# torognes/vsearch

Hardware: AMD Instinct MI355X
Metric: GCUPS (useful DP cells/s of the search16 global-alignment path: DP + traceback + CIGAR) (higher is better)
Workload: dtype int16

## Files before the change

### vsearch_amd/csrc/vsx_device.hip

```cpp
#include <hip/hip_runtime.h>
#include <type_traits>
#include <cstdlib>
#include <atomic>
#include "vsx_internal.h"

typedef unsigned int u32;
typedef unsigned int u32x4 __attribute__((ext_vector_type(4)));
typedef unsigned int u32x3 __attribute__((ext_vector_type(3)));
typedef short s2 __attribute__((ext_vector_type(2)));
typedef unsigned short us2 __attribute__((ext_vector_type(2)));

#define DEV __device__ __forceinline__
struct __attribute__((aligned(4))) Pair2 { unsigned int x, y; };

#define SIGN2 0x80008000u

DEV s2 S2(u32 x) { return __builtin_bit_cast(s2, x); }
DEV us2 U2(u32 x) { return __builtin_bit_cast(us2, x); }
DEV u32 UI(s2 x) { return __builtin_bit_cast(u32, x); }
DEV u32 UI(us2 x) { return __builtin_bit_cast(u32, x); }

DEV u32 sadd(u32 a, u32 b) { return UI(__builtin_elementwise_add_sat(S2(a), S2(b))); }
DEV u32 ssub(u32 a, u32 b) { return UI(__builtin_elementwise_sub_sat(S2(a), S2(b))); }
DEV u32 pmax(u32 a, u32 b) { return UI(__builtin_elementwise_max(S2(a), S2(b))); }
DEV u32 pmin(u32 a, u32 b) { return UI(__builtin_elementwise_min(S2(a), S2(b))); }
DEV u32 pminu(u32 a, u32 b) { return UI(__builtin_elementwise_min(U2(a), U2(b))); }
DEV u32 pmaxu(u32 a, u32 b) { return UI(__builtin_elementwise_max(U2(a), U2(b))); }
DEV u32 psubw(u32 a, u32 b) { return UI((us2) (U2(a) - U2(b))); }
DEV u32 pmad(u32 a, u32 b, u32 c) { return UI((us2) (U2(a) * U2(b) + U2(c))); }
DEV u32 pashr15(u32 a) { return UI((s2) (S2(a) >> (s2){15, 15})); }
DEV u32 bfi(u32 mask, u32 a, u32 b) { return (a & mask) | (b & ~mask); }
DEV u32 a_pk_minu(u32 a, u32 b) { u32 r; asm("v_pk_min_u16 %0, %1, %2" : "=v"(r) : "v"(a), "s"(b)); return r; }
DEV u32 a_pk_mad(u32 a, u32 b, u32 c) { u32 r; asm("v_pk_mad_u16 %0, %1, %2, %3" : "=v"(r) : "v"(a), "v"(b), "s"(c)); return r; }
DEV u32 a_bfi(u32 mask, u32 a, u32 b) { u32 r; asm("v_bfi_b32 %0, %1, %2, %3" : "=v"(r) : "s"(mask), "v"(a), "v"(b)); return r; }
DEV u32 a_bfi_v(u32 mask, u32 a, u32 b) { u32 r; asm("v_bfi_b32 %0, %1, %2, %3" : "=v"(r) : "v"(mask), "v"(a), "v"(b)); return r; }
DEV u32 a_lshr1(u32 a) { u32 r; asm("v_lshrrev_b32 %0, 1, %1" : "=v"(r) : "v"(a)); return r; }
DEV u32 a_pk_ashr15(u32 a) { u32 r; asm("v_pk_ashrrev_i16 %0, 15, %1 op_sel_hi:[0,1]" : "=v"(r) : "v"(a)); return r; }
DEV u32 funnel(u32 acc, u32 d) { return a_bfi(SIGN2, d, a_lshr1(acc)); }
DEV u32 pack16(int v) { const u32 x = (u32) v & 0xffffu; return x | (x << 16); }

DEV u32 dpp_shr1(u32 feed, u32 src) { return (u32) __builtin_amdgcn_update_dpp((int) feed, (int) src, 0x111, 0xF, 0xF, false); }
DEV u32 dpp_rol1(u32 src) { return (u32) __builtin_amdgcn_update_dpp((int) src, (int) src, 0x12F, 0xF, 0xF, false); }


#define VSX_COLCK_G 64
#define VSX_COLCK_DW(R_, lane_, block_) ((((size_t) ((lane_) / VSX_COLCK_G) * (size_t) ((2 * (R_)) / 4) + (size_t) (block_)) * VSX_COLCK_G + (size_t) ((lane_) % VSX_COLCK_G)) * 4)
#define VSX_RB 1
#define VSX_ROWCK_PAIR_DW(TILT_) ((TILT_) ? 192 : 256)
#define VSX_COLCK_NBH(RT_) (((RT_) + ((RT_) + 1) / 2 + 3) / 4)
#define VSX_COLCK_NB(R_, TILT_) ((TILT_) ? (VSX_MID(R_, true) ? 2 * VSX_COLCK_NBH((R_) / 2) : ((R_) + ((R_) + 1) / 2 + 3) / 4) : (2 * (R_)) / 4)
#ifndef VSX_CK_TASKMAJOR
#define VSX_CK_TASKMAJOR 1
#endif
#define VSX_CK_SLOT(TILT_, g_, l_) (((TILT_) && VSX_CK_TASKMAJOR) ? ((l_) * 4 + (g_)) : ((g_) * 16 + (l_)))
#ifndef VSX_COLCK_CG
#define VSX_COLCK_CG 64
#endif
#define VSX_CKT_BLOCK_DW 768
#define VSX_COLCK_NCHUNK(R_) ((VSX_COLCK_NB(R_, true) + 2) / 3)
#define VSX_COLCK_CDW(NB_, lane_, block_) ((((size_t) ((lane_) / VSX_COLCK_CG) * (size_t) (NB_) + (size_t) (block_)) * VSX_COLCK_CG + (size_t) ((lane_) % VSX_COLCK_CG)) * 4)
#ifndef VSX_FWD_WAVES
#define VSX_FWD_WAVES(R_, TILT_) ((R_) <= 16 ? 4 : ((R_) <= 24 ? 3 : 2))
#endif
#ifndef VSX_FWD_WAVES_ONE
#define VSX_FWD_WAVES_ONE(R_, TILT_) ((R_) == 26 ? 3 : VSX_FWD_WAVES(R_, TILT_))
#endif
typedef _Float16 f16x2 __attribute__((ext_vector_type(2)));
DEV u32 pk_max3_bits(u32 a, u32 b, u32 c)
{
  const f16x2 x = __builtin_bit_cast(f16x2, a), y = __builtin_bit_cast(f16x2, b), z = __builtin_bit_cast(f16x2, c);
  return __builtin_bit_cast(u32, __builtin_elementwise_maximum(__builtin_elementwise_maximum(x, y), z));
}
#ifndef VSX_FWD_WAVES_NQ
#define VSX_FWD_WAVES_NQ(R_, NQ_) ((NQ_) == 4 ? 2 : ((R_) <= 24 ? 3 : 2))
#endif
template <int R, bool GENERIC, bool TRACK, bool CKPT, bool TILT = false, bool MAX3 = false, int NQ = 1, bool PAIR = false, bool ONE = false>
__global__ void __launch_bounds__(PAIR ? 256 : 64) __attribute__((amdgpu_waves_per_eu(NQ == 1 ? (ONE ? VSX_FWD_WAVES_ONE(R, TILT) : VSX_FWD_WAVES(R, TILT)) : VSX_FWD_WAVES_NQ(R, NQ), 8)))
vsx_forward_kernel(const VsxDevParams P, const VsxTask * __restrict__ tasks,
                   const uint8_t * __restrict__ qc, const uint8_t * __restrict__ tc,
                   u32 * __restrict__ dir, uint2 * strip, VsxSlotOut * __restrict__ slot_out, const u32 ntasks)
{
  constexpr int ND = (R + 3) / 4;
  constexpr bool TOPPAD = CKPT && GENERIC && !TRACK;
  static_assert(!TILT || TOPPAD, "tilted coordinates exist for the TOPPAD class only");
  const int tl = TILT ? P.tilt : 0;
  static_assert(!MAX3 || TILT, "the MAX3 arithmetic is a sub-class of TILT");
  constexpr u32 BIAS16 = MAX3 ? 0x3E00u : (TILT ? 0x8000u : 0u);
  constexpr u32 BIAS = BIAS16 * 0x10001u;
  constexpr u32 CK_REBIAS = 0u;
  auto bpack = [](int v) -> u32 { return pack16(v + (int) BIAS16); };
  auto vadd = [](u32 a, u32 b) -> u32 { return TILT ? a + b : sadd(a, b); };
  auto vsubk = [](u32 a, u32 b) -> u32 { return TILT ? a - b : ssub(a, b); };
  auto vsub = [](u32 a, u32 b) -> u32 { return TILT ? psubw(a, b) : ssub(a, b); };
  auto vmax = [](u32 a, u32 b) -> u32 { return TILT ? pmaxu(a, b) : pmax(a, b); };
  constexpr bool MIDCK = VSX_MID(R, TILT);
  constexpr int RT = MIDCK ? R / 2 : R;
  constexpr bool CKST = TILT && (VSX_CKT != 0);
  static_assert(!(MAX3 && CKST), "the transposed A/B layout predates the MAX3 class");
  constexpr bool QPL = TILT && (VSX_QPL != 0);
  constexpr bool QP8 = CKST || QPL;
  constexpr int RP = (R + 3) & ~3;
  static_assert(NQ == 1 || NQ == 2 || NQ == 4, "tasks per wave");
  static_assert(NQ == 1 || (TILT && VSX_QPL != 0 && !VSX_CKT), "the sparse-task classes exist for the look-ahead TILT kernels only");
  static_assert(!PAIR || (NQ == 1 && TILT && VSX_QPL != 0 && VSX_FEED2 != 0 && !VSX_CKT && GENERIC), "the pair-profile classes extend the FEED2 look-ahead kernels");
  constexpr int WPB = PAIR ? 4 : 1;
  constexpr int QPBYTES = 16 * 16 * RP;
  constexpr int RPP = ((RP / 4) & 1) ? RP : RP + 4;
  __shared__ __attribute__((aligned(16))) u32 PPf[PAIR ? 16 * 16 * RPP : 4];
  __shared__ __attribute__((aligned(16))) int16_t QP[(GENERIC && !PAIR) ? (QP8 ? (NQ * QPBYTES) / 2 : 16 * 16 * R) : 8];
  uint8_t * const QPb = reinterpret_cast<uint8_t *>(QP);
  __shared__ __attribute__((aligned(16))) u32 RS[CKST ? 64 * 12 : 4];
  constexpr int FSZ = (TILT && VSX_QPL ? 2 : 1) * 4 * 16;
  __shared__ uint4 FEED4a[FSZ * WPB];
  __shared__ u32 FEEDFa[FSZ * WPB], FEEDN[GENERIC ? 1 : 4 * 16];
  constexpr bool FEED2 = (VSX_FEED2 != 0) && TOPPAD && (TILT && (VSX_QPL != 0));
  __shared__ uint2 FEEDBa[FEED2 ? 2 * 4 * 16 * WPB : 1];

  const int wv = PAIR ? __builtin_amdgcn_readfirstlane((int) (threadIdx.x >> 6)) : 0;
  uint4 * const FEED4 = FEED4a + wv * FSZ;
  u32 * const FEEDF = FEEDFa + wv * FSZ;
  uint2 * const FEEDB = FEEDBa + (FEED2 ? wv * FSZ : 0);
  const int lane = PAIR ? (int) (threadIdx.x & 63) : (int) threadIdx.x;
  const int gw = lane >> 4;
  constexpr int GPT = 4 / NQ;
  const int sq = (NQ == 1) ? 0 : gw / GPT;
  const int g = (NQ == 1) ? gw : gw % GPT;
  const int l = lane & 15;
  const u32 tix = PAIR ? blockIdx.x * 4u + (u32) wv : ((NQ == 1) ? blockIdx.x : blockIdx.x * (u32) NQ + (u32) sq);
  const bool sub_on = (NQ == 1 && !PAIR) ? true : (tix < ntasks);
  const VsxTask & T = tasks[sub_on ? tix : ntasks - 1];
  uint8_t * const QPl = reinterpret_cast<uint8_t *>(QP) + ((NQ == 1) ? 0 : sq * QPBYTES);

  const int Q = (int) T.qlen;
  const int total_lanes = (Q + R - 1) / R;
  const int rcnt0 = Q - (total_lanes - 1) * R;
  const int rc0 = __builtin_amdgcn_readfirstlane(rcnt0);
  static_assert(!PAIR || ONE, "the pair-profile classes are planned for single-strip queries only");
  const int nstrips = (NQ == 1 && !ONE) ? (total_lanes + 15) >> 4 : 1;
  const int steps = (NQ == 1) ? (int) T.steps : __builtin_amdgcn_readfirstlane((int) T.steps);

  const int DA = sub_on ? (int) T.tlen[2 * g] : 0;
  const int DB = sub_on ? (int) T.tlen[2 * g + 1] : 0;
  const int DpA = (DA + 3) & ~3;
  const int DpB = (DB + 3) & ~3;
  const int Dpg = DpA > DpB ? DpA : DpB;
  const uint8_t * __restrict__ tA = tc + T.toff[2 * g];
  const uint8_t * __restrict__ tB = tc + T.toff[2 * g + 1];
  const uint8_t * __restrict__ qq = qc + T.qoff;

  const u32 qrt_i_pk = pack16(P.qrt_i);
  u32 hmin = 0, hmax = 0;
  u32 score = 0;
  u32 lv1 = 0xFFFFFFFFu, leave = 0;

  for (int s = 0; s < nstrips; ++s)
    {
      const int L = 16 * s + l;
      const bool lane_on = (L < total_lanes) && (Dpg > 0);
      const bool first = (L == 0);
      const int pad = TOPPAD ? R - rcnt0 : 0;
      const int i0 = first ? -pad : rcnt0 + (L - 1) * R;

      if (GENERIC)
        {
          __syncthreads();
          if (PAIR)
            {
              for (int idx = (int) threadIdx.x; idx < 16 * 16 * RP; idx += 256)
                {
                  const int pr = idx / (16 * RP), row = idx % (16 * RP);
                  const int Lr = 16 * s + row / RP, rr = row % RP;
                  int va = 0, vb = 0;
                  if (rr < R)
                    {
                      if (Lr == 0 && rr < pad) va = vb = -P.top_step + 2 * tl;
                      else if (Lr < total_lanes)
                        {
                          const int gi = (Lr == 0) ? rr - pad : rcnt0 + (Lr - 1) * R + rr;
                          const int qs = (int) qq[gi];
                          va = P.matrix[(1 << (pr >> 2)) * 16 + qs];
                          vb = P.matrix[(1 << (pr & 3)) * 16 + qs];
                        }
                    }
                  PPf[(pr * 16 + row / RP) * RPP + rr] = ((u32) va & 0xffu) | (((u32) vb & 0xffu) << 16);
                }
            }
          else if (QP8)
            {
              constexpr int LPT = 64 / NQ;
              for (int idx = (NQ == 1) ? lane : lane % LPT; idx < 16 * 16 * RP; idx += LPT)
                {
                  const int code = idx / (16 * RP), row = idx % (16 * RP);
                  const int Lr = 16 * s + row / RP, rr = row % RP;
                  int v = 0;
                  if (rr < R)
                    {
                      if (Lr == 0 && rr < pad) v = -P.top_step + 2 * tl;
                      else if (Lr < total_lanes)
                        {
                          const int gi = (Lr == 0) ? rr - pad : rcnt0 + (Lr - 1) * R + rr;
                          v = P.matrix[code * 16 + (int) qq[gi]];
                        }
                    }
                  QPl[idx] = (uint8_t) v;
                }
            }
          else
          for (int idx = lane; idx < 16 * 16 * R; idx += 64)
            {
              const int code = idx / (16 * R), row = idx % (16 * R);
              const int Lr = 16 * s + row / R, rr = row % R;
              int v = 0;
              if (TOPPAD && Lr == 0 && rr < pad) v = -P.top_step + 2 * tl;
              else if (Lr < total_lanes && (TOPPAD || !(Lr == 0 && rr >= rcnt0)))
                {
                  const int gi = (Lr == 0) ? rr - pad : rcnt0 + (Lr - 1) * R + rr;
                  v = P.matrix[code * 16 + (int) qq[gi]];
                }
              QP[idx] = (int16_t) v;
            }
          __syncthreads();
        }

      u32 hprev[R];
      u32 hnext[R];
      u32 E[R];
      u32 ac[R];
#pragma unroll
      for (int r = 0; r < R; ++r)
        {
          int i = i0 + r;
          const bool dummy = TOPPAD && first && r < pad;
          if (i > Q - 1) i = Q - 1;
          if (i < 0) i = 0;
          const u32 a = qq[i];
          ac[r] = a | (a << 16);
          u32 hl = bpack(P.hleft[i]);
          u32 e0 = vsub(hl, (i < Q - 1) ? P.qrq_i_pk : P.qrq_r_pk);
          if (dummy)
            {
              const int sh = (r - pad - 1) * tl;
              hl = bpack(((r == pad - 1) ? 0 : -P.top_open) + sh);
              e0 = vsub(bpack(-P.top_open - P.top_step + sh), P.qrq_i_pk);
            }
          hprev[r] = hl;
          hnext[r] = hl;
          E[r] = e0;
        }
      u32 diag = first ? bpack(((TOPPAD && pad > 0) ? -P.top_open : 0) - (pad + 2) * tl) : bpack(P.hleft[i0 - 1]);
      const bool lastpos = (L == total_lanes - 1);
      const u32 qrq_last = lastpos ? P.qrq_r_pk : P.qrq_i_pk;
      const u32 rq_last = lastpos ? P.rq_r_pk : P.rq_i_pk;

      u32 sym = 0, nd = 0, qrt = 0, rt = 0;
      u32 symf = 0;
      u32 outH = 0, outF = 0;
      u32 f_sym = 0, f_nd = 0, f_qrt = 0, f_rt = 0, f_H = 0, f_F = 0;
      u32 rawA = 0, rawB = 0;
      int rawH = 0;
      uint2 rawS = make_uint2(0, 0);
      const uint2 * strip_in = strip + T.strip_off + (size_t) (((s + 1) & 1) * 4 + g) * (size_t) steps;
      uint2 * strip_outp = strip + T.strip_off + (size_t) ((s & 1) * 4 + g) * (size_t) steps;

      auto prefetch = [&](int blk) {
        const int c = 16 * blk + l;
        rawA = (c < DA) ? (u32) tA[c] : 0u;
        rawB = (c < DB) ? (u32) tB[c] : 0u;
        if (s == 0) rawH = P.htop[c];
        else if (c < Dpg) rawS = strip_in[c];
      };
      prefetch(0);

      auto build_feed = [&](int blk) __attribute__((always_inline)) {
              const int c = 16 * blk + l;
              auto mne = [&](u32 code) -> int {
                const bool unamb = (code != 0) && ((code & (code - 1)) == 0);
                return unamb ? P.mismatch : ((P.n_mismatch && code == 15) ? P.mismatch : 0);
              };
              const u32 ndA = (u32) (mne(rawA) - P.match) & 0xffffu;
              const u32 ndB = (u32) (mne(rawB) - P.match) & 0xffffu;
              const u32 qA = (u32) ((c < DA - 1) ? P.qrt_i : P.qrt_r) & 0xffffu;
              const u32 qB = (u32) ((c < DB - 1) ? P.qrt_i : P.qrt_r) & 0xffffu;
              const u32 rA = (u32) ((c < DA - 1) ? P.rt_i : P.rt_r) & 0xffffu;
              const u32 rB = (u32) ((c < DB - 1) ? P.rt_i : P.rt_r) & 0xffffu;
              const u32 sA = rawA | ((c == DA - 1) ? 0x100u : 0u) | ((c < DpA) ? 0x200u : 0u);
              const u32 sB = rawB | ((c == DB - 1) ? 0x100u : 0u) | ((c < DpB) ? 0x200u : 0u);
              f_sym = sA | (sB << 16);
              f_nd = ndA | (ndB << 16);
              f_qrt = qA | (qB << 16);
              f_rt = rA | (rB << 16);
              if (s == 0)
                {
                  f_H = bpack(rawH - pad * tl);
                  f_F = vsub(f_H, f_qrt);
                }
              else
                {
                  f_H = rawS.x;
                  f_F = rawS.y;
                }
              const int fo = QPL ? (blk & 1) * 64 : 0;
              if (FEED2)
                {
                  const u32 f_off = PAIR ? (((rawA >> 1) - (rawA >> 3)) * 4u + ((rawB >> 1) - (rawB >> 3))) * (u32) (16 * RPP * 4)
                                         : (rawA * (u32) (16 * RP) | ((rawB * (u32) (16 * RP)) << 16));
                  FEED4[fo + gw * 16 + l] = make_uint4(f_off, f_sym, f_H, f_F);
                  FEEDB[fo + gw * 16 + l] = make_uint2(f_qrt, f_rt);
                }
              else
                {
                  FEED4[fo + gw * 16 + l] = make_uint4(f_sym, f_qrt, f_rt, f_H);
                  FEEDF[fo + gw * 16 + l] = f_F;
                }
              if (!GENERIC) FEEDN[gw * 16 + l] = f_nd;
              prefetch(blk + 1);
      };
      constexpr int PD = RP / 4;
      u32 profA[2][(QPL && !PAIR) ? PD : 1], profB[2][(QPL && !PAIR) ? PD : 1];
      auto load_profile = [&](u32 (&buf)[2][(QPL && !PAIR) ? PD : 1], u32 sy) __attribute__((always_inline)) {
        if (PAIR) return;
        const u32 cd = sy & 0x000F000Fu;
        constexpr int QPA = (RP % 16 == 0) ? 16 : ((RP % 8 == 0) ? 8 : 4);
        if (FEED2)
          {
            const uint8_t * pa = QPl + l * RP + (sy & 0xFFFFu);
            const uint8_t * pb = QPl + l * RP + (sy >> 16);
            constexpr int PDN = (QPL && !PAIR) ? PD : 1;
            if constexpr (PAIR) { }
            else if constexpr (QPA == 16)
              {
#pragma unroll
                for (int k = 0; k < PDN; k += 4)
                  {
                    const uint4 va = *reinterpret_cast<const uint4 *>(pa + 4 * k), vb = *reinterpret_cast<const uint4 *>(pb + 4 * k);
                    buf[0][k] = va.x; buf[0][k + 1] = va.y; buf[0][k + 2] = va.z; buf[0][k + 3] = va.w;
                    buf[1][k] = vb.x; buf[1][k + 1] = vb.y; buf[1][k + 2] = vb.z; buf[1][k + 3] = vb.w;
                  }
              }
            else if constexpr (QPA == 8)
              {
#pragma unroll
                for (int k = 0; k < PDN; k += 2)
                  {
                    const uint2 va = *reinterpret_cast<const uint2 *>(pa + 4 * k), vb = *reinterpret_cast<const uint2 *>(pb + 4 * k);
                    buf[0][k] = va.x; buf[0][k + 1] = va.y;
                    buf[1][k] = vb.x; buf[1][k + 1] = vb.y;
                  }
              }
            else
              {
#pragma unroll
                for (int k = 0; k < PDN; ++k)
                  { buf[0][k] = reinterpret_cast<const u32 *>(pa)[k]; buf[1][k] = reinterpret_cast<const u32 *>(pb)[k]; }
              }
            return;
          }
        const u32 * a = reinterpret_cast<const u32 *>(QPl + (cd & 0xFu) * (16 * RP) + l * RP);
        const u32 * b = reinterpret_cast<const u32 *>(QPl + (cd >> 16) * (16 * RP) + l * RP);
#pragma unroll
        for (int k = 0; k < ((QPL && !PAIR) ? PD : 1); ++k) { buf[0][k] = a[k]; buf[1][k] = b[k]; }
      };
      if (QPL)
        {
          build_feed(0);
          sym = dpp_shr1(FEED4[gw * 16].x, 0u);
          load_profile(profA, sym);
        }

      const uint4 * const feed4_g = FEED4 + gw * 16;
      const u32 * const feedf_g = FEEDF + gw * 16;
      u32 pendH = 0, pendF = 0;
      u32 jpk_run = 0;
      u32 pendMH = 0, pendMF = 0, curMH = 0, curMF = 0;
      bool pend_on = false;
      const size_t ck_rowdw = ((((size_t) nstrips * steps + 1) & ~(size_t) 1) >> 1) * VSX_ROWCK_PAIR_DW(TILT);
      const size_t ck_nblk = ((size_t) steps + 15) >> 4;
      constexpr int CK_LANE_DW = TILT ? 3 : 4;
      constexpr size_t CK_COL_DW = TILT ? (size_t) 64 * 4 * VSX_COLCK_NB(R, true) : (size_t) 64 * (2 * R);
      const int ck_slot = VSX_CK_SLOT(TILT, gw, l);
      u32 * const rck_base = dir + T.dir_off + ((((size_t) s * steps) >> 1) * 64 + ck_slot) * CK_LANE_DW;
      u32 * const cck_base = dir + T.dir_off + ck_rowdw + (size_t) s * ck_nblk * CK_COL_DW;
      u32 * const mck_base = dir + T.dir_off + ck_rowdw + (size_t) nstrips * ck_nblk * CK_COL_DW
                             + ((((size_t) s * steps) >> 1) * 64 + ck_slot) * CK_LANE_DW;
      u32 * const rck_blk = dir + T.dir_off + (((size_t) s * steps) >> 3) * VSX_CKT_BLOCK_DW;
      u32 * const cck_blk = dir + T.dir_off + (((size_t) nstrips * steps) >> 3) * VSX_CKT_BLOCK_DW
                            + (size_t) s * ck_nblk * VSX_COLCK_NCHUNK(R) * VSX_CKT_BLOCK_DW;
      auto flush_block = [&](u32 * gdst) __attribute__((always_inline)) {
        __syncthreads();
#pragma unroll
        for (int k = 0; k < 3; ++k)
          {
            const u32x4 v = *reinterpret_cast<const u32x4 *>(RS + (k * 64 + lane) * 4);
            __builtin_nontemporal_store(v, reinterpret_cast<u32x4 *>(gdst + (k * 64 + lane) * 4));
          }
        __syncthreads();
      };

      auto step = [&](const int t, u32 (&hin)[R], u32 (&hout)[R], u32 (&pc)[2][(QPL && !PAIR) ? PD : 1], u32 (&pn)[2][(QPL && !PAIR) ? PD : 1],
                      auto interior_tag, auto odd_tag, auto steady_tag) __attribute__((always_inline)) {
          constexpr bool INTERIOR = decltype(interior_tag)::value;
          constexpr bool ODD = decltype(odd_tag)::value;
          constexpr bool STEADY = decltype(steady_tag)::value;
          u32 symn = 0;
          u32 pp[PAIR ? RP : 1];
          if (PAIR)
            {
              const u32 * ppa = PPf + (sym >> 2) + l * RPP;
#pragma unroll
              for (int k = 0; k < (PAIR ? RP : 0); k += 4)
                {
                  const uint4 v = *reinterpret_cast<const uint4 *>(ppa + k);
                  pp[k] = v.x; pp[k + 1] = v.y; pp[k + 2] = v.z; pp[k + 3] = v.w;
                }
            }
          if (QPL) { if ((t & 15) == 15) build_feed((t >> 4) + 1); }
          else if ((t & 15) == 0) build_feed(t >> 4);

          const int fo = QPL ? ((t >> 4) & 1) * 64 : 0;
          const u32 fslot = (u32) (fo + (t & 15));
          const uint4 fv = feed4_g[fslot];
          const u32 fF = FEED2 ? fv.w : feedf_g[fslot];
          if (QPL)
            {
              const int t1 = t + 1;
              symn = dpp_shr1(feed4_g[(u32) (((t1 >> 4) & 1) * 64 + (t1 & 15))].x, sym);
              load_profile(pn, symn);
            }
          else sym = dpp_shr1(fv.x, sym);
          if (!GENERIC) nd = dpp_shr1(FEEDN[gw * 16 + (t & 15)], nd);
          if (!INTERIOR)
            {
              if (FEED2)
                {
                  const uint2 fb = FEEDB[fo + gw * 16 + (t & 15)];
                  qrt = dpp_shr1(fb.x, qrt); rt = dpp_shr1(fb.y, rt);
                  symf = dpp_shr1(fv.y, symf);
                }
              else { qrt = dpp_shr1(fv.y, qrt); rt = dpp_shr1(fv.z, rt); }
            }
          const u32 inH = dpp_shr1(FEED2 ? fv.z : fv.w, outH);
          const u32 inF = dpp_shr1(fF, outF);

          const int j = t - l;
          const bool active = STEADY ? true : (lane_on && j >= 0 && j < Dpg);
          if (active)
            {
              const u32 code = sym & 0x000F000Fu;
              const int16_t * qpA = QP + (code & 0xFu) * (16 * R) + l * R;
              const int16_t * qpB = QP + (code >> 16) * (16 * R) + l * R;
              u32 pa = 0, pb = 0;
              u32 Hd = diag;
              u32 F = inF;
              u32 smn = 0x7FFF7FFFu, smx = 0x80008000u;
              u32 acc = 0, h2 = 0;
              u32 capH = 0, capF = 0, capmn = 0, capmx = 0;
              u32 dw[ND];
              u32 lastL = 0, lastEL = 0;
              u32 midH = 0, midF = 0;
              auto rows = [&](auto shared_tag) __attribute__((always_inline)) {
              constexpr bool SHARED = decltype(shared_tag)::value;
              constexpr bool LASTFAST = MAX3 && SHARED && CKPT;
#pragma unroll
              for (int r = 0; r < R; ++r)
                {
                  u32 V;
                  if (PAIR) V = pp[r];
                  else if (GENERIC && QP8)
                    {
                      if ((r & 3) == 0)
                        {
                          if (QPL) { pa = pc[0][r >> 2]; pb = pc[1][r >> 2]; }
                          else
                            {
                              pa = *reinterpret_cast<const u32 *>(QPb + (code & 0xFu) * (16 * RP) + l * RP + r);
                              pb = *reinterpret_cast<const u32 *>(QPb + (code >> 16) * (16 * RP) + l * RP + r);
                            }
                        }
                      V = __builtin_amdgcn_perm(pb, pa, 0x0C040C00u + 0x00010001u * (u32) (r & 3));
                    }
                  else if (GENERIC)
                    {
                      if (R % 2 == 0)
                        {
                          if ((r & 3) == 0 && r + 3 < R)
                            {
                              typedef typename std::conditional<R % 4 == 0, uint2, Pair2>::type Rows4;
                              const Rows4 va = *reinterpret_cast<const Rows4 *>(qpA + r);
                              const Rows4 vb = *reinterpret_cast<const Rows4 *>(qpB + r);
                              pa = va.x; pb = vb.x;
                              ac[r + 1] = va.y; ac[r + 2] = vb.y;
                            }
                          else if ((r & 3) == 0)
                            {
                              pa = *reinterpret_cast<const u32 *>(qpA + r);
                              pb = *reinterpret_cast<const u32 *>(qpB + r);
                            }
                          else if ((r & 3) == 2) { pa = ac[r - 1]; pb = ac[r]; }
                          V = (r & 1) ? __builtin_amdgcn_perm(pb, pa, 0x07060302u) : __builtin_amdgcn_perm(pb, pa, 0x05040100u);
                        }
                      else V = (u32) (uint16_t) qpA[r] | ((u32) (uint16_t) qpB[r] << 16);
                    }
                  else V = a_pk_mad(a_pk_minu(ac[r] ^ code, 0x00010001u), nd, P.match_pk);
                  const u32 h0 = vadd(Hd, V);
                  const bool ONE_MAX = MAX3 && (r < R - 1 || LASTFAST);
                  const u32 h1 = ONE_MAX ? 0u : vmax(h0, F);
                  h2 = ONE_MAX ? pk_max3_bits(h0, F, E[r]) : vmax(h1, E[r]);
                  if (TRACK) { smn = pmin(smn, h2); smx = pmax(smx, h2); }
                  Hd = hin[r];
                  hout[r] = h2;
                  const u32 qrq = (r == R - 1) ? qrq_last : P.qrq_i_pk;
                  const u32 rq = (r == R - 1) ? rq_last : P.rq_i_pk;
                  const u32 he = (r < R - 1) ? vsubk(h2, qrq) : vsub(h2, qrq);
                  const u32 hf = (SHARED && r < R - 1) ? he : vsub(h2, qrt);
                  const u32 f = (TILT && INTERIOR) ? F : vsub(F, rt);
                  const u32 e = (TILT && INTERIOR && r < R - 1) ? E[r] : vsub(E[r], rq);
                  if (CKPT && r == R - 1) { lastL = LASTFAST ? 0u : vsub(h1, E[r]); lastEL = vsub(he, e); }
                  if (!CKPT)
                    {
                      const u32 dU = ssub(h0, F);
                      const u32 dL = ssub(h1, E[r]);
                      const u32 dEU = ssub(hf, f);
                      const u32 dEL = ssub(he, e);
                      acc = funnel(funnel(funnel(funnel(acc, dU), dL), dEU), dEL);
                      if ((r & 3) == 3 || r == R - 1) dw[r >> 2] = acc;
                    }
                  F = vmax(f, hf);
                  E[r] = vmax(e, he);
                  if (MIDCK && r == RT - 1) { midH = h2; midF = F; }
                  if (!TOPPAD && __builtin_expect(rc0 == r + 1, 0)) { capH = h2; capF = F; capmn = smn; capmx = smx; }
                }
              };
              if (INTERIOR) rows(std::true_type {});
              else rows(std::false_type {});
              const u32 hl = (!TOPPAD && first) ? capH : h2;
              F = (!TOPPAD && first) ? capF : F;
              smn = (!TOPPAD && first) ? capmn : smn;
              smx = (!TOPPAD && first) ? capmx : smx;
              outH = hl;
              outF = F;
              diag = inH;
              if (CKPT)
                {
                  const u32 jpk = STEADY ? jpk_run : ((u32) j | ((u32) j << 16));
                  if (STEADY) jpk_run += 0x00010001u;
                  if (!INTERIOR)
                    {
                      const u32 atlast = a_pk_ashr15((FEED2 ? symf : sym) << 7);
                      leave = a_bfi_v(atlast, a_bfi_v(a_pk_ashr15(lastL), lv1, jpk), leave);
                    }
                  lv1 = a_bfi_v(a_pk_ashr15((MAX3 && INTERIOR) ? lastEL : (lastL | lastEL)), lv1, jpk);
                }

              if (TRACK)
                {
                  const u32 vm = a_pk_ashr15(sym << 6);
                  hmin = pmin(hmin, a_bfi_v(vm, smn, 0x7FFF7FFFu));
                  hmax = pmax(hmax, a_bfi_v(vm, smx, 0x80008000u));
                }
              if (!INTERIOR)
                {
                  const u32 lm = a_pk_ashr15((FEED2 ? symf : sym) << 7);
                  score = a_bfi_v(lm, hl, score);
                }

              const size_t gt = (size_t) s * steps + t;
              if (CKPT)
                {
                  if (!ODD) { pendH = outH; pendF = outF; }
                  if (MIDCK) { if (!ODD) { pendMH = midH; pendMF = midF; } else { curMH = midH; curMF = midF; } }
                }
              else
                {
                  u32 * dp = dir + T.dir_off + (((gt >> 2) * 64 + lane) * 4 + (gt & 3)) * ND;
                  if (ND == 4) *reinterpret_cast<uint4 *>(dp) = make_uint4(dw[0], dw[1], dw[2], dw[3]);
                  else if (ND == 2) *reinterpret_cast<uint2 *>(dp) = make_uint2(dw[0], dw[1]);
                  else
                    {
#pragma unroll
                      for (int w = 0; w < ND; ++w) dp[w] = dw[w];
                    }
                }
              if (l == 15 && s + 1 < nstrips) strip_outp[j] = make_uint2(outH, outF);
            }
          if (CKPT && CKST)
            {
              if (!ODD) pend_on = active;
              else
                {
                  const u32 dpk = __builtin_amdgcn_perm(psubw(outH, outF), psubw(pendH, pendF), 0x06040200u);
                  u32 * rs = RS + ck_slot * 12;
                  const int i = t & 7;
                  *reinterpret_cast<uint2 *>(rs + (i - 1)) = make_uint2(pendH, outH);
                  rs[8 + (i >> 1)] = dpk;
                  if (i == 7) flush_block(rck_blk + (size_t) (t >> 3) * VSX_CKT_BLOCK_DW);
                }
            }
          else if (CKPT)
            {
              if (!ODD) pend_on = active;
              else if (pend_on || active)
                {
                  if (TILT && !CKST)
                    {
                      const u32 dpk = __builtin_amdgcn_perm(psubw(outH, outF), psubw(pendH, pendF), 0x06040200u);
                      __builtin_nontemporal_store((u32x3) {pendH + CK_REBIAS, outH + CK_REBIAS, dpk}, reinterpret_cast<u32x3 *>(rck_base + (size_t) (t >> 1) * 192));
                      if (MIDCK)
                        {
                          const u32 dpm = __builtin_amdgcn_perm(psubw(curMH, curMF), psubw(pendMH, pendMF), 0x06040200u);
                          __builtin_nontemporal_store((u32x3) {pendMH + CK_REBIAS, curMH + CK_REBIAS, dpm}, reinterpret_cast<u32x3 *>(mck_base + (size_t) (t >> 1) * 192));
                        }
                    }
                  else
                    __builtin_nontemporal_store((u32x4) {pendH, pendF, outH, outF}, reinterpret_cast<u32x4 *>(rck_base + (size_t) (t >> 1) * 256));
                }
            }
          if (CKPT && (t & 15) == 15)
            {
              u32 * cb = cck_base + (size_t) (t >> 4) * CK_COL_DW;
              if (TILT)
                {
                  constexpr int NF = R + (R + 1) / 2;
                  constexpr int NFH = RT + (RT + 1) / 2, ZH = 4 * VSX_COLCK_NBH(RT);
                  auto flatc = [&](int z) -> u32 {
                    if (MIDCK)
                      {
                        const int hh = z / ZH, zz = z % ZH, r00 = hh * RT;
                        if (zz < RT) return hout[r00 + zz] + CK_REBIAS;
                        if (zz < NFH)
                          {
                            const int r0 = r00 + 2 * (zz - RT), r1 = (r0 + 1 < r00 + RT) ? r0 + 1 : r0;
                            return __builtin_amdgcn_perm(psubw(hout[r1], E[r1]), psubw(hout[r0], E[r0]), 0x06040200u);
                          }
                        return 0u;
                      }
                    if (z < R) return hout[z] + CK_REBIAS;
                    if (z < NF)
                      {
                        const int r0 = 2 * (z - R), r1 = r0 + 1 < R ? r0 + 1 : r0;
                        return __builtin_amdgcn_perm(psubw(hout[r1], E[r1]), psubw(hout[r0], E[r0]), 0x06040200u);
                      }
                    return 0u;
                  };
                  if (CKST)
                    {
                      constexpr int NBC = VSX_COLCK_NB(R, true);
#pragma unroll
                      for (int c = 0; c < VSX_COLCK_NCHUNK(R); ++c)
                        {
#pragma unroll
                          for (int pc = 0; pc < 3; ++pc)
                            {
                              const int z = 4 * (3 * c + pc);
                              if (3 * c + pc < NBC)
                                *reinterpret_cast<u32x4 *>(RS + ck_slot * 12 + pc * 4) = (u32x4) {flatc(z), flatc(z + 1), flatc(z + 2), flatc(z + 3)};
                            }
                          flush_block(cck_blk + ((size_t) (t >> 4) * VSX_COLCK_NCHUNK(R) + c) * VSX_CKT_BLOCK_DW);
                        }
                    }
                  else
                    {
#pragma unroll
                  for (int z = 0; z < 4 * VSX_COLCK_NB(R, true); z += 4)
                    __builtin_nontemporal_store((u32x4) {flatc(z), flatc(z + 1), flatc(z + 2), flatc(z + 3)}, reinterpret_cast<u32x4 *>(cb + VSX_COLCK_CDW(VSX_COLCK_NB(R, true), ck_slot, z >> 2)));
                    }
                }
              else if (R % 2 == 0)
                {
                  auto flat = [&](int z) -> u32 { return z < R ? hout[z] : E[z - R]; };
#pragma unroll
                  for (int z = 0; z < 2 * R; z += 4)
                    __builtin_nontemporal_store((u32x4) {flat(z), flat(z + 1), flat(z + 2), flat(z + 3)}, reinterpret_cast<u32x4 *>(cb + VSX_COLCK_DW(R, lane, z >> 2)));
                }
              else
                {
                  u32 * cp = cb + lane * (2 * R);
#pragma unroll
                  for (int x = 0; x < R; ++x) { cp[x] = hout[x]; cp[R + x] = E[x]; }
                }
            }
          if (QPL) sym = symn;
      };
      int t_switch = 0;
      if (CKPT && P.share_sub)
        {
          int dmin = 0x7fffffff;
          if (DA > 0 && DA < dmin) dmin = DA;
          if (DB > 0 && DB < dmin) dmin = DB;
#pragma unroll
          for (int m = 32; m >= 1; m >>= 1) { const int o = __shfl_xor(dmin, m, 64); dmin = o < dmin ? o : dmin; }
          t_switch = __builtin_amdgcn_readfirstlane(dmin == 0x7fffffff ? 0 : dmin - 1) & ~1;
          if (t_switch > steps) t_switch = steps & ~1;
        }
      int t = 0;
      qrt = qrt_i_pk; rt = pack16(P.rt_i);
      for (; t < t_switch && (TRACK || t < 16); t += 2)
        {
          step(t, hprev, hnext, profA, profB, std::true_type {}, std::false_type {}, std::false_type {});
          step(t + 1, hnext, hprev, profB, profA, std::true_type {}, std::true_type {}, std::false_type {});
        }
      if (!TRACK)
        for (jpk_run = (u32) (t - l) * 0x00010001u; t < t_switch; t += 2)
          {
            step(t, hprev, hnext, profA, profB, std::true_type {}, std::false_type {}, std::true_type {});
            step(t + 1, hnext, hprev, profB, profA, std::true_type {}, std::true_type {}, std::true_type {});
          }
      for (; t < steps; t += 2)
        {
          step(t, hprev, hnext, profA, profB, std::false_type {}, std::false_type {}, std::false_type {});
          step(t + 1, hnext, hprev, profB, profA, std::false_type {}, std::true_type {}, std::false_type {});
        }

      if (s + 1 < nstrips)
        {
          __builtin_amdgcn_fence(__ATOMIC_RELEASE, "agent");
          __builtin_amdgcn_fence(__ATOMIC_ACQUIRE, "agent");
        }
    }

#pragma unroll
  for (int m = 8; m >= 1; m >>= 1)
    {
      hmin = pmin(hmin, (u32) __shfl_xor((int) hmin, m, 16));
      hmax = pmax(hmax, (u32) __shfl_xor((int) hmax, m, 16));
    }
  const int l_last = (total_lanes - 1) & 15;
  score = (u32) __shfl((int) score, l_last, 16);
  leave = (u32) __shfl((int) leave, l_last, 16);
  if (l == 0)
    {
      const int mnA = (int16_t) (hmin & 0xffff), mnB = (int16_t) (hmin >> 16);
      const int mxA = (int16_t) (hmax & 0xffff), mxB = (int16_t) (hmax >> 16);
      VsxSlotOut oA, oB;
      score = psubw(score, BIAS);
      oA.score = (int16_t) ((int) (int16_t) (score & 0xffff) - (DA > 0 ? (Q + DA - 2) * tl : 0));
      oB.score = (int16_t) ((int) (int16_t) (score >> 16) - (DB > 0 ? (Q + DB - 2) * tl : 0));
      oA.leave = (uint16_t) (leave & 0xffff); oB.leave = (uint16_t) (leave >> 16); oA.pad = 0; oB.pad = 0;
      oA.overflow = (mnA <= P.smin || mxA >= 32767) ? 1 : 0;
      oB.overflow = (mnB <= P.smin || mxB >= 32767) ? 1 : 0;
      if (sub_on)
        {
          slot_out[(size_t) tix * VSX_TASK_SLOTS + 2 * g] = oA;
          slot_out[(size_t) tix * VSX_TASK_SLOTS + 2 * g + 1] = oB;
        }
    }
}

__global__ void __launch_bounds__(256)
vsx_traceback_kernel(const VsxDevParams P, const VsxTask * __restrict__ tasks,
                     const u32 * __restrict__ pair_slot, const u32 * __restrict__ pair_ids, u32 npairs,
                     const uint8_t * __restrict__ qc, const uint8_t * __restrict__ tc,
                     const u32 * __restrict__ dir, const VsxSlotOut * __restrict__ slot,
                     u32 * __restrict__ slab, const uint64_t * __restrict__ slab_off,
                     u32 * __restrict__ runs, uint64_t runs_capacity, unsigned long long * cursor,
                     VsxPairOut * __restrict__ out)
{
  const u32 k = blockIdx.x * blockDim.x + threadIdx.x;
  if (k >= npairs) return;
  const u32 ts = pair_slot[k];
  const u32 task = ts >> 3, sl = ts & 7;
  const VsxTask & T = tasks[task];
  const VsxSlotOut so = slot[ts];

  VsxPairOut o;
  o.pad = 0;
  o.nruns = 0;
  o.run_off = 0;
  if (so.overflow)
    {
      o.score = 32767; o.aligned = 0; o.matches = 0; o.mismatches = 0; o.gaps = 0;
      out[pair_ids[k]] = o;
      return;
    }

  const int R = (int) T.rows;
  const int ND = (R + 3) >> 2;
  const int Q = (int) T.qlen;
  const int D = (int) T.tlen[sl];
  const int total_lanes = (Q + R - 1) / R;
  const int rcnt0 = Q - (total_lanes - 1) * R;
  const size_t steps = T.steps;
  const int g = (int) (sl >> 1) + (int) T.group0;
  const bool hi = (sl & 1) != 0;
  const uint8_t * __restrict__ q = qc + T.qoff;
  const uint8_t * __restrict__ d = tc + T.toff[sl];
  u32 * __restrict__ my = slab + slab_off[k];

  int i = Q - 1, j = D - 1;
  int L = total_lanes - 1;
  int r = (L == 0 ? rcnt0 : R) - 1;
  int op = -1;
  u32 runlen = 0, nruns = 0;
  u32 al = 0, ma = 0, mi = 0, ga = 0;

  auto push = [&](int newop) {
    if (newop == op) { ++runlen; return; }
    if (op >= 0) my[nruns++] = (runlen << 2) | (u32) op;
    op = newop;
    runlen = 1;
  };
  auto row_up = [&]() {
    --i;
    if (--r < 0) { --L; r = (L == 0 ? rcnt0 : R) - 1; }
  };

  while (i >= 0 && j >= 0)
    {
      const int s = L >> 4, l = L & 15;
      const size_t t = (size_t) j + (size_t) l;
      const size_t gt = (size_t) s * steps + t;
      const u32 w = dir[T.dir_off + (((gt >> 2) * 64 + (size_t) (g * 16 + l)) * 4 + (gt & 3)) * ND + (size_t) (r >> 2)];
      const u32 hw = hi ? (w >> 16) : (w & 0xffffu);
      int rid = R - 4 * (r >> 2);
      if (rid > 4) rid = 4;
      const int pos = 16 - 4 * rid + 4 * (r & 3);
      const u32 b = (hw >> pos) & 15u;
      ++al;
      if (op == 1 && (b & 8u)) { --j; push(1); }
      else if (op == 2 && (b & 4u)) { row_up(); push(2); }
      else if (b & 2u) { if (op != 1) ++ga; --j; push(1); }
      else if (b & 1u) { if (op != 2) ++ga; row_up(); push(2); }
      else
        {
          const u32 a = q[i], c = d[j];
          if ((a & c) != 0 && !(P.n_mismatch && (a == 15 || c == 15))) ++ma; else ++mi;
          row_up(); --j; push(0);
        }
    }
  while (i >= 0) { ++al; if (op != 2) ++ga; --i; push(2); }
  while (j >= 0) { ++al; if (op != 1) ++ga; --j; push(1); }
  if (op >= 0) my[nruns++] = (runlen << 2) | (u32) op;

  const unsigned long long base = atomicAdd(cursor, (unsigned long long) nruns);
  if (base + nruns <= runs_capacity)
    for (u32 x = 0; x < nruns; ++x) runs[base + x] = my[x];

  o.score = so.score;
  o.aligned = (uint16_t) al; o.matches = (uint16_t) ma; o.mismatches = (uint16_t) mi; o.gaps = (uint16_t) ga;
  o.nruns = nruns;
  o.run_off = base;
  out[pair_ids[k]] = o;
}

DEV u32 half_lo(u32 w, bool hi) { return hi ? (w >> 16) : w; }
DEV int wave_max_i32(int v)
{
#pragma unroll
  for (int m = 32; m >= 1; m >>= 1) { const int o = __shfl_xor(v, m, 64); v = o > v ? o : v; }
  return v;
}

DEV void rank_note(const VsxFilterDev & FL, u32 pid, u32 verdict, int score, double idv)
{
  if (FL.rank_counts == nullptr) return;
  if (verdict == 1u || verdict == 2u)
    {
      const u32 pos = atomicAdd(FL.rank_counts, 1u);
      FL.kept_pair[pos] = pid;
      FL.kept_id[pos] = idv;
// ... 1401 lines not shown
```

Baseline: 7971.

## Unroll steady-state loop by 16 with lean feed build and scalar column index

The steady interior loop is unrolled into 16-step blocks. In those blocks the feed is rebuilt through a lean path that only writes the profile offsets and the H/F seeds, skipping the mismatch, gap and symbol-flag packing. The per-lane running column register is replaced by a scalar step counter fed to v_bfi with an SGPR operand, and lv1 is biased by the lane index before the loop and unbiased after it. A VALU-budget profiling script is also added. The lean feed relies on the interior steps never reading the skipped fields, and the 16-step unroll may raise code size and register pressure.

```diff
diff --git a/profiles/valu_budget.py b/profiles/valu_budget.py
--- /dev/null
+++ b/profiles/valu_budget.py
@@ -0,0 +1,184 @@
+#!/usr/bin/env python3
+import argparse
+import collections
+import os
+import re
+import shutil
+import subprocess
+import sys
+import tempfile
+
+LLVM = "/opt/rocm/llvm/bin"
+ROOT = os.path.dirname(os.path.dirname(os.path.abspath(__file__)))
+
+
+def mangled(args):
+    a = [x.strip() for x in args.split(",")]
+    enc = "".join(("Li%sE" % x) if x.lstrip("-").isdigit() else ("Lb%dE" % (x == "true")) for x in a)
+    return "_Z18vsx_forward_kernelI" + enc + "Ev12VsxDevParamsPK7VsxTaskPKhS5_PjP15HIP_vector_typeIjLj2EEP10VsxSlotOutj"
+
+
+def extract(lib, sym, tmp):
+    shutil.copy(lib, os.path.join(tmp, "lib.so"))
+    subprocess.run([LLVM + "/llvm-objdump", "--offloading", "lib.so"], cwd=tmp, capture_output=True, check=True)
+    for f in sorted(os.listdir(tmp)):
+        if "gfx950" not in f:
+            continue
+        p = os.path.join(tmp, f)
+        syms = subprocess.run([LLVM + "/llvm-readelf", "-s", "--wide", p], capture_output=True, text=True).stdout
+        if (" " + sym + "\n") in syms:
+            return p, syms
+    sys.exit("kernel %s not found in %s" % (sym, lib))
+
+
+def meta(syms, sym):
+    out = {}
+    for k in ("num_vgpr", "numbered_sgpr", "private_seg_size"):
+        m = re.search(r"\s([0-9a-f]+)\s+0\s+NOTYPE\s+LOCAL\s+DEFAULT\s+ABS\s+" + re.escape(sym) + r"\." + k + r"\n", syms)
+        out[k] = int(m.group(1), 16) if m else None
+    m = re.search(r"\s([0-9a-f]+)\s+(\d+)\s+FUNC\s+\S+\s+\S+\s+\S+\s+" + re.escape(sym) + r"\n", syms)
+    out["start"], out["size"] = int(m.group(1), 16), int(m.group(2))
+    return out
+
+
+def disasm(co, sym, start):
+    txt = subprocess.run([LLVM + "/llvm-objdump", "-d", "--mcpu=gfx950", "--disassemble-symbols=" + sym, co],
+                         capture_output=True, text=True, check=True).stdout
+    ins = []
+    for line in txt.splitlines():
+        m = re.match(r"\s+(\S+)\s*(.*?)\s*//\s*([0-9A-F]+):", line)
+        if not m:
+            continue
+        op, rest, addr = m.group(1), m.group(2), int(m.group(3), 16) - start
+        t = re.search(r"<" + re.escape(sym) + r"\+0x([0-9a-f]+)>", line)
+        ins.append((addr, op, rest, int(t.group(1), 16) if t else None))
+    return ins
+
+
+def is_valu(op):
+    return op.startswith("v_")
+
+
+def category(op, rest):
+    if op in ("v_pk_maximum3_f16", "v_pk_max_u16", "v_subrev_u32_e32", "v_sub_u32_e32", "v_subrev_u32_e64", "v_sub_u32_e64"):
+        return "row body"
+    if op == "v_mov_b32_dpp":
+        return "DPP hand-overs (feed, H, F)"
+    if op == "v_add_u32_sdwa":
+        return "profile row addresses"
+    if op in ("v_pk_ashrrev_i16", "v_bfi_b32"):
+        return "leave-column tracking"
+    if op in ("v_lshl_add_u32", "v_lshlrev_b32_e32", "v_or_b32_e32", "v_and_or_b32") and "s" in rest.split(",")[1]:
+        return "feed-slot addresses"
+    if op in ("v_lshl_add_u64", "v_add_co_u32_e32", "v_addc_co_u32_e32", "v_mad_u64_u32"):
+        return "checkpoint addresses"
+    if op == "v_mov_b32_e32":
+        return "register copies"
+    return None
+
+
+def budget(body, R, S):
+    c = collections.Counter()
+    quota = {"v_perm_b32": R * S, "v_add_u32_e32": R * S}
+    npk = sum(1 for op, _ in body if op == "v_pk_sub_i16")
+    nashr = sum(1 for op, _ in body if op == "v_pk_ashrrev_i16")
+    pk = [("row body", S), ("last row's own e / hf subtractions", 2 * S), ("leave-column tracking", nashr)]
+    for op, rest in body:
+        if not is_valu(op):
+            continue
+        k = category(op, rest)
+        if k is None and op in quota:
+            if op == "v_add_u32_e32" and re.search(r"0x(1|2)000(1|2)\b", rest):
+                k = "leave-column tracking"
+            elif quota[op] > 0:
+                quota[op] -= 1
+                k = "row body"
+            else:
+                k = "checkpoint pack" if op == "v_perm_b32" else "other"
+        if k is None and op == "v_pk_sub_i16":
+            for i, (name, n) in enumerate(pk):
+                if n > 0:
+                    pk[i] = (name, n - 1)
+                    k = name
+                    break
+            else:
+                k = "checkpoint pack"
+        c[k or "other"] += 1
+    return c, npk
+
+
+def main():
+    ap = argparse.ArgumentParser()
+    ap.add_argument("--lib", default=os.path.join(ROOT, "vsearch_amd", "libvsx.so"))
+    ap.add_argument("--kernel", default="16,true,false,true,true,true,1,false,true", help="template arguments of vsx_forward_kernel")
+    ap.add_argument("--rows", type=int, default=None, help="R (default: the first template argument)")
+    ap.add_argument("--loop", type=int, default=None, help="loop index to budget (default: most v_pk_maximum3_f16)")
+    ap.add_argument("--ops", action="store_true", help="print the opcode histogram of the loop too")
+    a = ap.parse_args()
+    R = a.rows or int(a.kernel.split(",")[0])
+    sym = mangled(a.kernel)
+    tmp = tempfile.mkdtemp(prefix="vsx_budget_")
+    try:
+        co, syms = extract(a.lib, sym, tmp)
+        md = meta(syms, sym)
+        ins = disasm(co, sym, md["start"])
+    finally:
+        shutil.rmtree(tmp, ignore_errors=True)
+    print("vsx_forward_kernel<%s>  (%s)" % (a.kernel, os.path.relpath(a.lib, ROOT) if a.lib.startswith(ROOT) else a.lib))
+    print("  code %d B, %d instructions, %d VALU;  VGPR %s  SGPR %s  scratch %s B" % (
+        md["size"], len(ins), sum(is_valu(op) for _, op, _, _ in ins), md["num_vgpr"], md["numbered_sgpr"], md["private_seg_size"]))
+    idx = {addr: k for k, (addr, _, _, _) in enumerate(ins)}
+    heads = collections.OrderedDict()
+    for k, (addr, op, _, tgt) in enumerate(ins):
+        if op.startswith("s_branch") or op.startswith("s_cbranch"):
+            if tgt is not None and tgt <= addr and tgt in idx:
+                h = idx[tgt]
+                heads.setdefault(h, []).append(k)
+    loops = []
+    for h, bs in heads.items():
+        first_back, last = min(bs), max(bs)
+        main_path = set(range(h, first_back + 1))
+        for k in range(h, first_back + 1):
+            addr, op, _, tgt = ins[k]
+            if op.startswith("s_cbranch") and tgt is not None and tgt > addr and tgt in idx and idx[tgt] <= first_back + 1:
+                for j in range(k + 1, idx[tgt]):
+                    main_path.discard(j)
+        cond = [j for j in range(h, last + 1) if j not in main_path]
+        mp = sorted(main_path)
+        loops.append(dict(head=h, end=last, main=mp, cond=cond,
+                          max3=sum(1 for j in mp if ins[j][1] == "v_pk_maximum3_f16"),
+                          valu_main=sum(1 for j in mp if is_valu(ins[j][1])), valu_cond=sum(1 for j in cond if is_valu(ins[j][1]))))
+    print("  loops (offset range: VALU on the always-taken path + in branch-guarded regions, v_pk_maximum3_f16):")
+    for n, L in enumerate(loops):
+        print("    [%d] +0x%04x..+0x%04x: %4d + %4d VALU, %3d max3" % (n, ins[L["head"]][0], ins[L["end"]][0], L["valu_main"], L["valu_cond"], L["max3"]))
+    if not loops:
+        return
+    n = a.loop if a.loop is not None else max(range(len(loops)), key=lambda i: (loops[i]["max3"], -i))
+    L = loops[n]
+    S = max(1, round(L["max3"] / R))
+    body = [(ins[j][1], ins[j][2]) for j in L["main"]]
+    cond = [(ins[j][1], ins[j][2]) for j in L["cond"]]
+    cm, _ = budget(body, R, S)
+    per_step = L["valu_main"] / S + L["valu_cond"] / 16.0
+    print("  loop [%d]: %d steps per iteration (R = %d)" % (n, S, R))
+    print("    VALU per two steps, always-taken path: %.1f" % (2.0 * L["valu_main"] / S))
+    print("    VALU in branch-guarded regions (once per 16 steps): %d" % L["valu_cond"])
+    print("    VALU per 16-step block: %.0f   per step: %.2f   (row body %d per step = %.1f %%)" % (
+        16 * per_step, per_step, 6 * R, 100.0 * 6 * R / per_step))
+    print("    per step, by category (always-taken path / S, + branch-guarded / 16):")
+    order = ["row body", "DPP hand-overs (feed, H, F)", "profile row addresses", "feed-slot addresses", "last row's own e / hf subtractions",
+             "leave-column tracking", "checkpoint pack", "checkpoint addresses", "register copies", "other"]
+    for k in order:
+        v = cm.get(k, 0) / S
+        if v:
+            print("      %-38s %6.2f" % (k, v))
+    if L["valu_cond"]:
+        print("      %-38s %6.2f  (%d VALU / 16)" % ("16-step block boundary (guarded)", L["valu_cond"] / 16.0, L["valu_cond"]))
+    if a.ops:
+        for name, lst in (("always-taken path", body), ("branch-guarded", cond)):
+            h = collections.Counter(op for op, _ in lst if is_valu(op))
+            print("    %s opcodes: %s" % (name, ", ".join("%s %d" % kv for kv in h.most_common())))
+
+
+if __name__ == "__main__":
+    main()
diff --git a/vsearch_amd/csrc/vsx_device.hip b/vsearch_amd/csrc/vsx_device.hip
--- a/vsearch_amd/csrc/vsx_device.hip
+++ b/vsearch_amd/csrc/vsx_device.hip
@@ -34,6 +34,7 @@
 DEV u32 a_pk_mad(u32 a, u32 b, u32 c) { u32 r; asm("v_pk_mad_u16 %0, %1, %2, %3" : "=v"(r) : "v"(a), "v"(b), "s"(c)); return r; }
 DEV u32 a_bfi(u32 mask, u32 a, u32 b) { u32 r; asm("v_bfi_b32 %0, %1, %2, %3" : "=v"(r) : "s"(mask), "v"(a), "v"(b)); return r; }
 DEV u32 a_bfi_v(u32 mask, u32 a, u32 b) { u32 r; asm("v_bfi_b32 %0, %1, %2, %3" : "=v"(r) : "v"(mask), "v"(a), "v"(b)); return r; }
+DEV u32 a_bfi_vs(u32 mask, u32 a, u32 b) { u32 r; asm("v_bfi_b32 %0, %1, %2, %3" : "=v"(r) : "v"(mask), "v"(a), "s"(b)); return r; }
 DEV u32 a_lshr1(u32 a) { u32 r; asm("v_lshrrev_b32 %0, 1, %1" : "=v"(r) : "v"(a)); return r; }
 DEV u32 a_pk_ashr15(u32 a) { u32 r; asm("v_pk_ashrrev_i16 %0, 15, %1 op_sel_hi:[0,1]" : "=v"(r) : "v"(a)); return r; }
 DEV u32 funnel(u32 acc, u32 d) { return a_bfi(SIGN2, d, a_lshr1(acc)); }
@@ -271,8 +272,19 @@
       };
       prefetch(0);
 
-      auto build_feed = [&](int blk) __attribute__((always_inline)) {
+      auto build_feed = [&](int blk, auto lean_tag) __attribute__((always_inline)) {
+              constexpr bool LEAN = FEED2 && decltype(lean_tag)::value;
               const int c = 16 * blk + l;
+              if (LEAN)
+                {
+                  f_H = (s == 0) ? bpack(rawH - pad * tl) : rawS.x;
+                  f_F = (s == 0) ? vsub(f_H, qrt_i_pk) : rawS.y;
+                  const u32 f_off = PAIR ? (((rawA >> 1) - (rawA >> 3)) * 4u + ((rawB >> 1) - (rawB >> 3))) * (u32) (16 * RPP * 4)
+                                         : (rawA * (u32) (16 * RP) | ((rawB * (u32) (16 * RP)) << 16));
+                  FEED4[(blk & 1) * 64 + gw * 16 + l] = make_uint4(f_off, 0u, f_H, f_F);
+                  prefetch(blk + 1);
+                  return;
+                }
               auto mne = [&](u32 code) -> int {
                 const bool unamb = (code != 0) && ((code & (code - 1)) == 0);
                 return unamb ? P.mismatch : ((P.n_mismatch && code == 15) ? P.mismatch : 0);
@@ -362,7 +374,7 @@
       };
       if (QPL)
         {
-          build_feed(0);
+          build_feed(0, std::false_type {});
           sym = dpp_shr1(FEED4[gw * 16].x, 0u);
           load_profile(profA, sym);
         }
@@ -370,7 +382,6 @@
       const uint4 * const feed4_g = FEED4 + gw * 16;
       const u32 * const feedf_g = FEEDF + gw * 16;
       u32 pendH = 0, pendF = 0;
-      u32 jpk_run = 0;
       u32 pendMH = 0, pendMF = 0, curMH = 0, curMF = 0;
       bool pend_on = false;
       const size_t ck_rowdw = ((((size_t) nstrips * steps + 1) & ~(size_t) 1) >> 1) * VSX_ROWCK_PAIR_DW(TILT);
@@ -400,7 +411,8 @@
                       auto interior_tag, auto odd_tag, auto steady_tag) __attribute__((always_inline)) {
           constexpr bool INTERIOR = decltype(interior_tag)::value;
           constexpr bool ODD = decltype(odd_tag)::value;
-          constexpr bool STEADY = decltype(steady_tag)::value;
+          constexpr bool STEADY = decltype(steady_tag)::value != 0;
+          constexpr bool LEANFEED = decltype(steady_tag)::value == 2;
           u32 symn = 0;
           u32 pp[PAIR ? RP : 1];
           if (PAIR)
@@ -413,8 +425,8 @@
                   pp[k] = v.x; pp[k + 1] = v.y; pp[k + 2] = v.z; pp[k + 3] = v.w;
                 }
             }
-          if (QPL) { if ((t & 15) == 15) build_feed((t >> 4) + 1); }
-          else if ((t & 15) == 0) build_feed(t >> 4);
+          if (QPL) { if ((t & 15) == 15) build_feed((t >> 4) + 1, std::integral_constant<bool, LEANFEED> {}); }
+          else if ((t & 15) == 0) build_feed(t >> 4, std::false_type {});
 
           const int fo = QPL ? ((t >> 4) & 1) * 64 : 0;
           const u32 fslot = (u32) (fo + (t & 15));
@@ -541,14 +553,14 @@
               diag = inH;
               if (CKPT)
                 {
-                  const u32 jpk = STEADY ? jpk_run : ((u32) j | ((u32) j << 16));
-                  if (STEADY) jpk_run += 0x00010001u;
+                  const u32 jpk = (u32) j | ((u32) j << 16);
                   if (!INTERIOR)
                     {
                       const u32 atlast = a_pk_ashr15((FEED2 ? symf : sym) << 7);
                       leave = a_bfi_v(atlast, a_bfi_v(a_pk_ashr15(lastL), lv1, jpk), leave);
                     }
-                  lv1 = a_bfi_v(a_pk_ashr15((MAX3 && INTERIOR) ? lastEL : (lastL | lastEL)), lv1, jpk);
+                  const u32 lmask = a_pk_ashr15((MAX3 && INTERIOR) ? lastEL : (lastL | lastEL));
+                  lv1 = STEADY ? a_bfi_vs(lmask, lv1, (u32) t * 0x00010001u) : a_bfi_v(lmask, lv1, jpk);
                 }
 
               if (TRACK)
@@ -602,12 +614,13 @@
                 {
                   if (TILT && !CKST)
                     {
+                      const size_t ckp = LEANFEED ? (size_t) ((t & ~15) >> 1) * 192 + (size_t) (((t & 15) >> 1) * 192) : (size_t) (t >> 1) * 192;
                       const u32 dpk = __builtin_amdgcn_perm(psubw(outH, outF), psubw(pendH, pendF), 0x06040200u);
-                      __builtin_nontemporal_store((u32x3) {pendH + CK_REBIAS, outH + CK_REBIAS, dpk}, reinterpret_cast<u32x3 *>(rck_base + (size_t) (t >> 1) * 192));
+                      __builtin_nontemporal_store((u32x3) {pendH + CK_REBIAS, outH + CK_REBIAS, dpk}, reinterpret_cast<u32x3 *>(rck_base + ckp));
                       if (MIDCK)
                         {
                           const u32 dpm = __builtin_amdgcn_perm(psubw(curMH, curMF), psubw(pendMH, pendMF), 0x06040200u);
-                          __builtin_nontemporal_store((u32x3) {pendMH + CK_REBIAS, curMH + CK_REBIAS, dpm}, reinterpret_cast<u32x3 *>(mck_base + (size_t) (t >> 1) * 192));
+                          __builtin_nontemporal_store((u32x3) {pendMH + CK_REBIAS, curMH + CK_REBIAS, dpm}, reinterpret_cast<u32x3 *>(mck_base + ckp));
                         }
                     }
                   else
@@ -699,11 +712,26 @@
           step(t + 1, hnext, hprev, profB, profA, std::true_type {}, std::true_type {}, std::false_type {});
         }
       if (!TRACK)
-        for (jpk_run = (u32) (t - l) * 0x00010001u; t < t_switch; t += 2)
-          {
-            step(t, hprev, hnext, profA, profB, std::true_type {}, std::false_type {}, std::true_type {});
-            step(t + 1, hnext, hprev, profB, profA, std::true_type {}, std::true_type {}, std::true_type {});
-          }
+        {
+          const u32 lpk = (u32) l * 0x00010001u;
+          lv1 = psubw(lv1, psubw(0u, lpk));
+          for (; t + 32 <= t_switch; t += 16)
+            {
+              const int tb = t & ~15;
+#pragma unroll
+              for (int k = 0; k < 16; k += 2)
+                {
+                  step(tb + k, hprev, hnext, profA, profB, std::true_type {}, std::false_type {}, std::integral_constant<int, 2> {});
+                  step(tb + k + 1, hnext, hprev, profB, profA, std::true_type {}, std::true_type {}, std::integral_constant<int, 2> {});
+                }
+            }
+          for (; t < t_switch; t += 2)
+            {
+              step(t, hprev, hnext, profA, profB, std::true_type {}, std::false_type {}, std::true_type {});
+              step(t + 1, hnext, hprev, profB, profA, std::true_type {}, std::true_type {}, std::true_type {});
+            }
+          lv1 = psubw(lv1, lpk);
+        }
       for (; t < steps; t += 2)
         {
           step(t, hprev, hnext, profA, profB, std::false_type {}, std::false_type {}, std::false_type {});
```

New measurement: 8186, median of 6. +2.7%, better.
